# jmaronas/TGP.pytorch

Measured on AMD Instinct MI355X. Metric: ELBO-steps/sec (N x M kernel + chol + flow), Power M=100 S=32, higher is better.
Workload: dtype f64; 1 GPU; tgp_power_tanh3x2; rows_per_gpu=8611, D=4, M=100, S=32, flow=tanh3x2, parallelism=row-shard x1, launch=hipgraph, 40 / 10 steps per graph launch, replicas=1

## Files before the change

include/tgp_hip.h:

```cpp
#ifndef TGP_HIP_H
#define TGP_HIP_H

#include <stddef.h>
#include <stdint.h>

#ifdef __cplusplus
extern "C" {
#endif

#define TGP_VERSION 104
#define TGP_FUSED_MAX_M 128
#define TGP_BIG_MAX_M 4096

#define TGP_E_UNSUPPORTED (-100)
#define TGP_E_WORKSPACE (-101)
#define TGP_E_LDS (-102)
#define TGP_E_LAUNCH (-103)
#define TGP_E_COMM (-104)
#define TGP_STATUS_SYNC_TIMEOUT (-77)

#define TGP_FLOW_AFFINE 0
#define TGP_FLOW_SAL 1
#define TGP_FLOW_STEPTANH 2
#define TGP_FLOW_ARCSINH 3
#define TGP_FLOW_BOXCOX 4
#define TGP_FLOW_INV_BOXCOX 5
#define TGP_FLAG_RESTRICT 1
#define TGP_FLAG_ADD_F0 2
#define TGP_FLAG_PER_ROW 4

#define TGP_LIK_GAUSS 0
#define TGP_LIK_FLOW 1
#define TGP_LIK_ADJOINT 2
#define TGP_LIK_BERNOULLI 3
#define TGP_LIK_WARPED 4
#define TGP_LIK_SOFTMAX 5

#define TGP_KERNEL_SCALE_RBF 0
#define TGP_KERNEL_SCALE_MATERN32 1

#define TGP_PLAN_ROWS_AUTO 0
#define TGP_PLAN_ROWS_K16 1
#define TGP_PLAN_ROWS_K 2
#define TGP_PLAN_ROWS4_NW4 3
#define TGP_PLAN_ROWS4_NW8 4
#define TGP_PLAN_ROWS_MASK 15
#define TGP_PLAN_NO_CHUNK_OVERLAP 16
#define TGP_PLAN_CHUNK_ROWS(n) (((((n) + 127) / 128) & 0xffff) << 8)
#define TGP_PLAN_CHUNK_OF(plan) ((((plan) >> 8) & 0xffff) * 128)

typedef struct tgp_model {
  int32_t N;
  int32_t D;
  int32_t M;
  int32_t S;
  int32_t nblk;
  int32_t P;
  int32_t RP;
  int32_t lik;
  int32_t kernel;
  int32_t plan;
  double scale;
  double jitter;
  double kl_scale;
  double jitter_ladder;
  const double* Z;
  const double* raw_ls;
  const double* raw_os;
  const double* m;
  const double* Lam;
  const double* log_var_noise;
  const double* theta;
  const int32_t* program;
  const double* xs;
  const double* wn;
} tgp_model;

typedef struct tgp_grads {
  double* Z;
  double* raw_ls;
// ... 178 lines not shown
```

tgp/pytorch_amd/csrc/tgp_dev.hpp:

```cpp
#pragma once
#include <utility>
#include <hip/hip_runtime.h>
#include <stdint.h>
#include "../../../include/tgp_hip.h"

typedef double d4 __attribute__((ext_vector_type(4)));
#define TGP_MFMA(a, b, c) __builtin_amdgcn_mfma_f64_16x16x4f64((a), (b), (c), 0, 0, 0)

#define TGP_ROWS_PER_BLOCK 64
#define TGP_TILE_LD 66
#define TGP_MAX_MT 8
#ifndef TGP_RSPLIT
#define TGP_RSPLIT 4
#endif
#define TGP_LOG_2PI_REF 1.8378770942368803

#ifdef TGP_STAMPS
#define TGP_STAMP(wsp, plan, i)                                                                       \
  do {                                                                                                \
    if (blockIdx.x == 0 && threadIdx.x == 0)                                                          \
      (wsp)[(plan).hdr + tgp::H_STAMP + (i)] = (double)__builtin_amdgcn_s_memrealtime();              \
  } while (0)
#else
#define TGP_STAMP(wsp, plan, i) \
  do {                          \
  } while (0)
#endif

namespace tgp {

__device__ __forceinline__ void st_wt(double* p, double v) {
  __hip_atomic_store(p, v, __ATOMIC_RELAXED, __HIP_MEMORY_SCOPE_AGENT);
}

struct Plan {
  int N, D, M, S, nblk, P, RP, lik;
  int MT, MP, DP, CT, CT16, ntri, nblocks;
  int nw4;
  int rw;
  int rpb;
  int nslots;
  int zs_lds;
  size_t slab_G, slab_T, slab_S, slab_C, slab_len;
  size_t hdr, ils, ls, Zs, mpad, w, tp, tg;
  size_t Kmm, L, J, LT, Lq, LqT, S_, HpT, Q;
  size_t nD;
  size_t Gp;
  size_t redp;
  size_t PP;
  int PPW;
  size_t dbg;
  size_t slabs;
  size_t total;
};

enum { H_S2 = 0, H_KL = 1, H_ETA = 2, H_EINV = 3, H_SIG_OS = 4, H_STEP = 5, H_STAMP = 8, H_PSTAMP = 32, H_OUT = 60, H_N = 64 };
enum { C_ELL = 0, C_ETAB = 1, C_SVB = 2, C_PAD = 3, C_THETA = 4 };

inline size_t rup(size_t x, size_t a) { return (x + a - 1) / a * a; }

inline int rows4_waves(int N, int MT) {
  if ((N + 15) / 16 + MT <= 255) return 4;
  if ((N + 31) / 32 + MT <= 255) return 8;
  return 0;
}
inline int rows_rw(int N) { return (N > 4000 && (N + 39) / 40 <= 256) ? 10 : 16; }
inline int plan_alloc_blocks(int N) {
  int nb = (N + TGP_ROWS_PER_BLOCK - 1) / TGP_ROWS_PER_BLOCK;
  const int nw = rows4_waves(N, 1);
  if (nw > 0 && (N + 4 * nw - 1) / (4 * nw) > nb) nb = (N + 4 * nw - 1) / (4 * nw);
  const int rw = rows_rw(N);
  if ((N + 4 * rw - 1) / (4 * rw) > nb) nb = (N + 4 * rw - 1) / (4 * rw);
  return nb < 1 ? 1 : nb;
}

inline int make_plan(Plan& p, int N, int D, int M, int S, int nblk, int P, int RP, int lik, int nw4 = 0, int rw = 16) {
  if (D < 1 || D > 16) return -2;
  if (M < 1 || M > 16 * TGP_MAX_MT) return TGP_E_UNSUPPORTED;
  p.N = N; p.D = D; p.M = M; p.S = S; p.nblk = nblk; p.P = P; p.RP = RP; p.lik = lik; p.nslots = 0; p.zs_lds = 0;
  p.MT = (M + 15) / 16; p.MP = p.MT * 16;
  p.DP = D <= 4 ? 4 : (D <= 8 ? 8 : 16);
  p.CT = (2 * p.DP + 1 + 15) / 16; p.CT16 = p.CT * 16;
  p.ntri = p.MT * (p.MT + 1) / 2;
  p.nw4 = nw4;
  p.rw = rw;
  p.rpb = nw4 > 0 ? 4 * nw4 : 4 * rw;
  p.nblocks = (N + p.rpb - 1) / p.rpb;
  if (p.nblocks < 1) p.nblocks = 1;
  p.slab_G = 0;
  p.slab_T = p.slab_G + (size_t)p.ntri * 256;
  p.slab_S = p.slab_T + (size_t)p.MP * p.CT16;
  p.slab_C = p.slab_S + p.MP;
  p.slab_len = rup(p.slab_C + C_THETA + P, 16);
  size_t o = 0;
  const size_t mm = (size_t)p.MP * p.MP;
  p.hdr = o; o += H_N;
  p.ils = o; o += 16;
  p.ls = o; o += 16;
  p.Zs = o; o += (size_t)p.MP * p.DP;
  p.mpad = o; o += p.MP;
  p.w = o; o += p.MP;
  p.tp = o; o += rup(P + 1, 16);
  p.tg = o; o += rup(P + 1, 16);
  p.Kmm = o; o += mm; p.L = o; o += mm; p.J = o; o += mm; p.LT = o; o += mm;
  p.Lq = o; o += mm; p.LqT = o; o += mm; p.S_ = o; o += mm; p.HpT = o; o += mm; p.Q = o; o += mm;
  p.nD = o; o += (size_t)p.MT * 256;
  p.Gp = o; o += mm;
  p.redp = o; o += p.slab_len;
  p.PPW = p.DP + 2;
  p.PP = o; o += (size_t)2 * p.MT * p.MP * p.PPW;
  p.dbg = o; o += 256;
  p.slabs = o; o += (size_t)p.nblocks * p.slab_len;
  p.total = o;
  return 0;
}


__device__ __forceinline__ double exp_fast(double x) {
  x = fmin(fmax(x, -745.0), 709.0);
  const double k = rint(x * 1.4426950408889634074);
  double r = fma(-k, 6.93147180369123816490e-01, x);
  r = fma(-k, 1.90821492927058770002e-10, r);
  const double r2 = r * r, r4 = r2 * r2, r8 = r4 * r4;
  const double p01 = 1.0 + r;
  const double p23 = fma(r, 1.0 / 6.0, 0.5);
  const double p45 = fma(r, 1.0 / 120.0, 1.0 / 24.0);
  const double p67 = fma(r, 1.0 / 5040.0, 1.0 / 720.0);
  const double p89 = fma(r, 1.0 / 362880.0, 1.0 / 40320.0);
  const double pab = fma(r, 1.0 / 39916800.0, 1.0 / 3628800.0);
  const double pcd = fma(r, 1.0 / 6227020800.0, 1.0 / 479001600.0);
  const double q0 = fma(p23, r2, p01), q1 = fma(p67, r2, p45), q2 = fma(pab, r2, p89);
  const double s0 = fma(q1, r4, q0), s1 = fma(pcd, r4, q2);
  return ldexp(fma(s1, r8, s0), (int)k);
}

#define TGP_SQRT3 1.7320508075688772
__device__ __forceinline__ double cov_value(int kernel, double s2, double d2) {
  if (kernel == TGP_KERNEL_SCALE_MATERN32) {
    const double ar = TGP_SQRT3 * sqrt(fmax(d2, 1e-30));
    return s2 * (1.0 + ar) * exp_fast(-ar);
  }
  return s2 * exp_fast(-0.5 * d2);
}
__device__ __forceinline__ double cov_gweight(int kernel, double s2, double d2) {
// ... 1025 lines not shown
```

tgp/pytorch_amd/csrc/tgp_mm.hip:

```cpp
#include "tgp_dev.hpp"
#include "tgp_prep.hpp"
#include "tgp_launch.hpp"

namespace tgp {

#define PREP_THREADS 512
#ifndef TGP_W4_WINDOWS
#define TGP_W4_WINDOWS 2
#endif

__global__ __launch_bounds__(PREP_THREADS) void k_prep_a(Plan p, tgp_model md, FlowProg fp, double* __restrict__ ws,
                                                         int32_t* __restrict__ status) {
  extern __shared__ __attribute__((aligned(16))) unsigned char smem_raw[];
  double* sm = reinterpret_cast<double*>(smem_raw);
  const int tid = threadIdx.x, lane = tid & 63;
  const int wave = __builtin_amdgcn_readfirstlane(tid >> 6);
  const int r = lane & 15, q = lane >> 4;
  const int M = p.M, D = p.D, MP = p.MP, DP = p.DP, MT = p.MT;

  int32_t* sy = status + 4;
  const int nb_total = 3 + MT * MT;
  if ((int)blockIdx.x < MT * MT) {
    prep_tile_role<PREP_THREADS, true>(p, md, ws, (int)blockIdx.x, sy);
    sync_leave(sy, nb_total);
// ... 251 lines not shown
    __syncthreads();
    if (s_info == 0 || s_nan != 0 || !(md.jitter_ladder > 0.0) || attempt == 3) break;
    __syncthreads();
    if (tid == 0) s_info = 0;
    jit = md.jitter + md.jitter_ladder * (attempt == 0 ? 1.0 : (attempt == 1 ? 10.0 : 100.0));
    __syncthreads();
  }
  if (((MT - 1) & 1) == cb && wave == NW - 1) inv_diag(MT - 1);
  for (int t = wave; t < (MT + 1 - cb) / 2; t += NW) write_L(MT - 1, 2 * t + cb);
  PSTAMP(9);
#ifdef TGP_STAMPS
  if (lane == 0) {
    if (wave == 0)
      for (int i = 0; i < 10; ++i) ws[p.hdr + H_PSTAMP + i] = tph[i];
    if (wave == 3) for (int i = 1; i <= 5; ++i) { ws[p.hdr + H_PSTAMP + 26 + i] = tph[i]; ws[p.hdr + 20 + i] = tcnt[i]; }
    ws[p.hdr + H_PSTAMP + 10 + 2 * wave] = tph[7];
    ws[p.hdr + H_PSTAMP + 11 + 2 * wave] = tph[8];
  }
#endif
  if (tid == 0 && cb == 0) {
    status[0] = s_sync != 0 ? TGP_STATUS_SYNC_TIMEOUT : s_info;
    if (s_sync != 0) __hip_atomic_fetch_add(status + 3, 1, __ATOMIC_RELAXED, __HIP_MEMORY_SCOPE_AGENT);
    status[1] = s_nan;
    status[2] = s_info == 0 ? attempt : 0;
  }
  sync_leave(sy, nb_total);
#undef PREP_BARRIER
}

size_t prep_a_lds_bytes(const Plan& p) {
  return ((size_t)p.MP * (p.MP + 1) + (p.zs_lds ? (size_t)p.MP * p.DP : 0) + 16) * sizeof(double);
}

#define RED_ELEMS (256 / TGP_RSPLIT)
__global__ __launch_bounds__(256) void k_reduce(Plan p, double* __restrict__ ws) {
#ifdef TGP_STAMPS
  if (blockIdx.x == 0 && threadIdx.x == 0) ws[p.dbg + 200 + 16] = (double)__builtin_amdgcn_s_memrealtime();
#endif
  __shared__ double part_s[TGP_RSPLIT][RED_ELEMS];
  const int tid = threadIdx.x, sh = tid / RED_ELEMS, el = tid % RED_ELEMS;
  const size_t e = (size_t)blockIdx.x * RED_ELEMS + el;
  const bool in = e < p.slab_len;
  const int b0 = (int)((long long)p.nblocks * sh / TGP_RSPLIT), b1 = (int)((long long)p.nblocks * (sh + 1) / TGP_RSPLIT);
  const double* sl = ws + p.slabs + (in ? e : 0);
  constexpr int RB = 28;
  double s0 = 0.0, s1 = 0.0, s2 = 0.0, s3 = 0.0;
  for (int b = b0; b < b1; b += RB) {
    double t[RB];
#pragma unroll
    for (int u = 0; u < RB; ++u) {
      const int bu = b + u < b1 ? b + u : b1 - 1;
      t[u] = sl[(size_t)bu * p.slab_len];
    }
#pragma unroll
    for (int u = 0; u < RB; ++u) t[u] = b + u < b1 ? t[u] : 0.0;
#pragma unroll
    for (int u = 0; u < RB; u += 4) { s0 += t[u]; s1 += t[u + 1]; s2 += t[u + 2]; s3 += t[u + 3]; }
  }
  part_s[sh][el] = b1 > b0 ? (s0 + s1) + (s2 + s3) : 0.0;
  __syncthreads();
  if (sh != 0 || !in) return;
  double s = 0.0;
#pragma unroll
  for (int k = 0; k < TGP_RSPLIT; ++k) s += part_s[k][el];
  if (e < p.slab_T) {
    const int t = (int)(e >> 8), in_t = (int)(e & 255), row = in_t >> 4, col = in_t & 15;
    int ti = 0;
    while ((ti + 1) * (ti + 2) / 2 <= t) ++ti;
    const int tj = t - ti * (ti + 1) / 2;
    if (ti == tj && col > row) return;
    double* G = ws + p.Gp;
// ... 64 lines not shown
  }
  sv0 = tid < 16 ? red_tail(p, ws, p.slab_S + c0 + tid) : 0.0;
}
__device__ __forceinline__ void bwd_g_commit(const Plan& p, double* Gs, double* LbL, double* svL,
                                             const bwd_d2 (&gv)[BWD_G_NIT], double sv0) {
  const int MP = p.MP, tid = threadIdx.x;
#pragma unroll
  for (int u = 0; u < BWD_G_NIT; ++u) {
    const int i = tid + u * BWD_THREADS;
    if (i < MP * 8) {
      reinterpret_cast<bwd_d2*>(Gs)[i] = gv[u];
      reinterpret_cast<bwd_d2*>(LbL)[i] = bwd_d2{0.0, 0.0};
    }
  }
  if (tid < 16) svL[tid] = sv0;
}

template <int PF, bool SWAP = false, class FB>
__device__ __forceinline__ d4 tile_mm_regA(const double (&a)[PF], FB fb, int n, d4 acc) {
#pragma unroll
  for (int s0 = 0; s0 < PF; s0 += 8) {
    if (s0 < n) {
      double o[8];
#pragma unroll
      for (int u = 0; u < 8; ++u) o[u] = s0 + u < n ? fb(s0 + u) : 0.0;
#pragma unroll
      for (int u = 0; u < 8; ++u)
        if (s0 + u < n) acc = SWAP ? TGP_MFMA(o[u], a[s0 + u], acc) : TGP_MFMA(a[s0 + u], o[u], acc);
    }
  }
  return acc;
}

__device__ __forceinline__ void bwd_lam_role(const Plan& p, const tgp_model& md, const tgp_grads& g, double* __restrict__ ws,
                                             const AdamDev& ad, double* sm, int c, const int32_t* __restrict__ status) {
  static_assert(TGP_MAX_MT <= BWD_THREADS / 64, "one tile per wave");
  const int MP = p.MP, MT = p.MT, M = p.M;
  double* Gs = sm;
  double* LbL = Gs + (size_t)MP * 16;
  double* svL = LbL + (size_t)MP * 16;
  const int tid = threadIdx.x, lane = tid & 63, wave = __builtin_amdgcn_readfirstlane(tid >> 6), r = lane & 15, q = lane >> 4;
  const int c0 = 16 * c;
  BW_STAMP(c == 0, 4);
  bwd_d2 gv[BWD_G_NIT];
  double sv0;
  bwd_g_issue(p, ws, c0, gv, sv0);
  constexpr int PF = TGP_PF2;
  const double* __restrict__ Lq = ws + p.Lq;
  const int j = wave, j0 = 16 * j;
  const bool has = j < MT;
  const int n = has && j <= c ? (MP - j0) / 4 : 0;
  double lq[PF];
#pragma unroll
  for (int s_ = 0; s_ < PF; ++s_) lq[s_] = s_ < n ? Lq[(size_t)(j0 + 4 * s_ + q) * MP + j0 + r] : 0.0;
  const bool upd = ad.p != nullptr && !bwd_timed_out(status);
  const double step = upd ? (double)(ad.step_dev[0] + 1) : 1.0;
  double lamv[4], am[4], av[4];
  long ei[4];
#pragma unroll
  for (int rr = 0; rr < 4; ++rr) {
    const int row = c0 + r, col = j0 + q + 4 * rr;
    const bool in = has && row < M && col < M;
    const size_t e = in ? (size_t)row * M + col : 0;
    ei[rr] = in ? (long)e : -1;
    lamv[rr] = md.Lam[e];
    if (upd) { am[rr] = ad.m[ad.lam_off + e]; av[rr] = ad.v[ad.lam_off + e]; }
  }
  bwd_g_commit(p, Gs, LbL, svL, gv, sv0);
  __syncthreads();
  d4 acc = {0, 0, 0, 0};
  acc = tile_mm_regA<PF>(lq, [&](int s_) { return Gs[(j0 + 4 * s_ + q) * 16 + r]; }, n, acc);
  const double bc1 = 1.0 - exp_fast(step * ad.ln_b1), bc2s = sqrt(1.0 - exp_fast(step * ad.ln_b2));
#pragma unroll
  for (int rr = 0; rr < 4; ++rr) {
    if (ei[rr] < 0) continue;
    const int row = c0 + r, col = j0 + q + 4 * rr;
    double x = 0.0;
    if (col <= row) x = 2.0 * acc[rr] - md.kl_scale * (col == row ? lamv[rr] - 1.0 / lamv[rr] : lamv[rr]);
    g.Lam[ei[rr]] = x;
    if (upd) adam_elem(ad, ad.lam_off + ei[rr], x, ad.p[ad.lam_off + ei[rr]], am[rr], av[rr], bc1, bc2s);
  }
  BW_STAMP(c == 0, 5);
}

__device__ __forceinline__ void bwd_q_role(const Plan& p, double* __restrict__ ws, double* sm, int c, int32_t* sb) {
  static_assert(TGP_MAX_MT <= BWD_THREADS / 64, "one tile per wave");
  const int MP = p.MP, MT = p.MT;
  double* Gs = sm;
  double* LbL = Gs + (size_t)MP * 16;
  double* svL = LbL + (size_t)MP * 16;
  const int tid = threadIdx.x, lane = tid & 63, wave = __builtin_amdgcn_readfirstlane(tid >> 6), r = lane & 15, q = lane >> 4;
  const int c0 = 16 * c;
  BW_STAMP(c == 0, 0);
  bwd_d2 gv[BWD_G_NIT];
  double sv0;
  bwd_g_issue(p, ws, c0, gv, sv0);
  constexpr int PF = TGP_PF2;
  const double* __restrict__ HpT = ws + p.HpT;
  const double* __restrict__ Lm = ws + p.L;
  const double* __restrict__ w = ws + p.w;
  const bool has = wave < MT - c;
  const bool spare = MT - c < BWD_THREADS / 64, tw = spare && wave == MT - c;
  const int i0 = tw ? c0 : 16 * (c + wave);
  const int n1 = has ? MP / 4 : 0, n2 = has || tw ? (MP - i0) / 4 : 0;
  double hp[PF], pq[PF], wv[4];
#pragma unroll
  for (int s_ = 0; s_ < PF; ++s_) hp[s_] = s_ < n1 ? HpT[(size_t)(4 * s_ + q) * MP + i0 + r] : 0.0;
#pragma unroll
  for (int s_ = 0; s_ < PF; ++s_) pq[s_] = s_ < n2 ? Lm[(size_t)(i0 + 4 * s_ + q) * MP + i0 + r] : 0.0;
#pragma unroll
  for (int rr = 0; rr < 4; ++rr) wv[rr] = has ? w[i0 + q + 4 * rr] : 0.0;
  bwd_g_commit(p, Gs, LbL, svL, gv, sv0);
  __syncthreads();
  BW_STAMP(c == 0, 1);
  if (has) {
    d4 acc = {0, 0, 0, 0};
    acc = tile_mm_regA<PF>(hp, [&](int s_) { return Gs[(4 * s_ + q) * 16 + r]; }, n1, acc);
#pragma unroll
    for (int rr = 0; rr < 4; ++rr) {
      const int row = i0 + q + 4 * rr, col = c0 + r;
      LbL[row * 16 + r] = (col <= row) ? -(wv[rr] * svL[r] + 2.0 * acc[rr]) : 0.0;
    }
  }
  __syncthreads();
  BW_STAMP(c == 0, 2);
  double* Q = ws + p.Q;
  if (has) {
    d4 acc = {0, 0, 0, 0};
    acc = tile_mm_regA<PF>(pq, [&](int s_) { return LbL[(i0 + 4 * s_ + q) * 16 + r]; }, n2, acc);
    if (wave != 0) {
#pragma unroll
      for (int rr = 0; rr < 4; ++rr) {
        const int row = i0 + q + 4 * rr, col = c0 + r;
        st_agent(Q + (size_t)row * MP + col, acc[rr]);
        st_agent(Q + (size_t)col * MP + row, acc[rr]);
      }
    } else {
      d4 tr = {0, 0, 0, 0};
      if (!spare) tr = tile_mm_regA<PF, true>(pq, [&](int s_) { return LbL[(c0 + 4 * s_ + q) * 16 + r]; }, n2, tr);
#pragma unroll
      for (int rr = 0; rr < 4; ++rr) {
        const int rl = q + 4 * rr;
        if (r <= rl) st_agent(Q + (size_t)(c0 + rl) * MP + c0 + r, acc[rr]);
        else if (!spare) st_agent(Q + (size_t)(c0 + rl) * MP + c0 + r, tr[rr]);
      }
    }
  } else if (tw) {
    d4 tr = {0, 0, 0, 0};
    tr = tile_mm_regA<PF, true>(pq, [&](int s_) { return LbL[(c0 + 4 * s_ + q) * 16 + r]; }, n2, tr);
#pragma unroll
    for (int rr = 0; rr < 4; ++rr) {
      const int rl = q + 4 * rr;
      if (r > rl) st_agent(Q + (size_t)(c0 + rl) * MP + c0 + r, tr[rr]);
    }
  }
  handoff_barrier();
  if (tid == 0) sync_add(sb + SB_PROG, 1 << 16);
  BW_STAMP(c == 0, 3);
}

__device__ __forceinline__ void bwd_row_role(const Plan& p, double* __restrict__ ws, double* sm, int i, int h, int32_t* sb,
                                             int32_t* __restrict__ status) {
  static_assert(TGP_MAX_MT <= BWD_THREADS / 64, "one Y tile and one Ks tile per wave");
  const int MP = p.MP, MT = p.MT, DP = p.DP, PPW = p.PPW;
  const int tid = threadIdx.x, lane = tid & 63, wave = __builtin_amdgcn_readfirstlane(tid >> 6), r = lane & 15, q = lane >> 4;
  const int KH = (MT + 1) / 2, kb0 = h ? KH : 0, kb1 = h ? MT : KH, nk = kb1 - kb0;
  double* Yl = sm;
  double* zsL = Yl + (size_t)MT * 256;
  double* Ja = zsL + 16 * DP;
  const int i0 = 16 * i;
  const double* __restrict__ J = ws + p.J;
  const double* __restrict__ Q = ws + p.Q;
  BW_STAMP(i == 0 && h == 0, 6);
  double kmv[4];
  const int jbw = wave < MT ? wave : 0, j0w = 16 * jbw;
#pragma unroll
  for (int rr = 0; rr < 4; ++rr) kmv[rr] = (ws + p.Kmm)[(size_t)(i0 + q + 4 * rr) * MP + j0w + r];
  if (tid < 16 * DP) zsL[tid] = (ws + p.Zs)[(size_t)i0 * DP + tid];
  for (int e = tid; e < (MP - i0) * 16; e += BWD_THREADS) Ja[e] = J[(size_t)(i0 + (e >> 4)) * MP + i0 + (e & 15)];
  const int ks0 = 16 * (jbw > kb0 ? jbw : kb0), ks1 = 16 * kb1;
  const int n1 = wave < nk ? (MP - i0) / 4 : 0, n2 = wave < MT && ks1 > ks0 ? (ks1 - ks0) / 4 : 0;
  constexpr int PF = TGP_PF2, PFH = 2 * TGP_MAX_MT;
  double jb2[PFH];
#pragma unroll
  for (int s_ = 0; s_ < PFH; ++s_) jb2[s_] = s_ < n2 ? J[(size_t)(ks0 + 4 * s_ + q) * MP + j0w + r] : 0.0;
  __syncthreads();
  BW_STAMP(i == 0 && h == 0, 7);
  bwd_wait(sb + SB_PROG, [&](int x) { return ((x >> 16) & 0xff) >= MT; }, status);
  BW_STAMP(i == 0 && h == 0, 8);
  if (wave < nk) {
    d4 acc = {0, 0, 0, 0};
    double qv[PF];
#pragma unroll
    for (int s_ = 0; s_ < PF; ++s_) qv[s_] = s_ < n1 ? ld_agent(Q + (size_t)(i0 + 4 * s_ + q) * MP + 16 * (kb0 + wave) + r) : 0.0;
    acc = tile_mm_regA<PF, true>(qv, [&](int s_) { return Ja[(4 * s_ + q) * 16 + r]; }, n1, acc);
#pragma unroll
    for (int rr = 0; rr < 4; ++rr) Yl[wave * 256 + (q + 4 * rr) * 16 + r] = acc[rr];
  }
  __syncthreads();
  BW_STAMP(i == 0 && h == 0, 9);
  if (wave < MT) {
    d4 acc = {0, 0, 0, 0};
    acc = tile_mm_regA<PFH, true>(jb2, [&](int s_) { const int k = ks0 + 4 * s_; return Yl[((k >> 4) - kb0) * 256 + r * 16 + (k & 15) + q]; }, n2, acc);
    double ep[4];
#pragma unroll
    for (int rr = 0; rr < 4; ++rr) ep[rr] = 0.5 * acc[rr] * kmv[rr];
    double cs = quad_sum((ep[0] + ep[1]) + (ep[2] + ep[3]));
    double* out = ws + p.PP + (size_t)(2 * i + h) * PPW * MP + j0w + r;
    if (q == 0) st_agent(out + (size_t)DP * MP, cs);
    for (int d = 0; d < DP; ++d) {
      double s = 0.0;
#pragma unroll
      for (int rr = 0; rr < 4; ++rr) s += ep[rr] * zsL[(q + 4 * rr) * DP + d];
      s = quad_sum(s);
      if (q == 0) st_agent(out + (size_t)d * MP, s);
    }
  }
  handoff_barrier();
  if (tid == 0) sync_add(sb + SB_PROG, 1 << 24);
  BW_STAMP(i == 0 && h == 0, 10);
}

#define BWD_MIRROR_MAX 4096
#define BWDF_ADAM_PER_THREAD 2
__device__ __forceinline__ void bwd_final_role(const Plan& p, const tgp_model& md, const tgp_grads& g, double* __restrict__ out,
                                               double* __restrict__ ws, const AdamDev& ad, double* term, int32_t* sb,
                                               int32_t* __restrict__ status, int nb_total) {
// ... 92 lines not shown
      out[1] = timed_out ? nan_ : ell;
      out[2] = timed_out ? nan_ : kl;
      out[3] = 0.0;
    }
  }
  if (ad.p != nullptr && !timed_out) {
    if (mirror) __syncthreads();
    else handoff_barrier();
    const double bc1 = 1.0 - exp_fast(a_step * ad.ln_b1), bc2s = sqrt(1.0 - exp_fast(a_step * ad.ln_b2));
    auto grad = [&](long k, long i) { return mirror ? gl[k] : __hip_atomic_load(ad.g + i, __ATOMIC_RELAXED, __HIP_MEMORY_SCOPE_AGENT); };
#pragma unroll
    for (int u = 0; u < BWDF_ADAM_PER_THREAD; ++u) {
      const long k = tid + (long)NT * u;
      if (k < n_rest) {
        const long i = k < ad.lam_off ? k : k + ad.lam_n;
        adam_elem(ad, i, grad(k, i), ap[u], am[u], av[u], bc1, bc2s);
      }
    }
    for (long k = tid + (long)NT * BWDF_ADAM_PER_THREAD; k < n_rest; k += NT) {
      const long i = k < ad.lam_off ? k : k + ad.lam_n;
      adam_elem(ad, i, grad(k, i), ad.p[i], ad.m[i], ad.v[i], bc1, bc2s);
    }
  }
  BW_STAMP(true, 14);
  bwd_wait(sb + SB_LEFT, [&](int x) { return x >= nb_total - 1; }, status);
  __syncthreads();
  if (tid == 0) {
    sync_st(sb + SB_PROG, 0); sync_st(sb + SB_LEFT, 0);
    if (ad.p != nullptr && !timed_out) atomicAdd(&ad.step_dev[0], 1);
  }
  BW_STAMP(true, 15);
}

__global__ __launch_bounds__(BWD_THREADS) void k_bwd(Plan p, tgp_model md, tgp_grads g, double* __restrict__ out,
                                                     double* __restrict__ ws, AdamDev ad, int32_t* __restrict__ status) {
  extern __shared__ __attribute__((aligned(16))) unsigned char smem_raw[];
  double* sm = reinterpret_cast<double*>(smem_raw);
  const int MT = p.MT, b = (int)blockIdx.x;
  int32_t* sb = status + 6;
  if (b < MT) {
    bwd_q_role(p, ws, sm, b, sb);
    bwd_leave(sb);
  } else if (b < 2 * MT) {
    bwd_lam_role(p, md, g, ws, ad, sm, b - MT, status);
    bwd_leave(sb);
  } else if (b < 4 * MT) {
    bwd_row_role(p, ws, sm, (b - 2 * MT) >> 1, (b - 2 * MT) & 1, sb, status);
    bwd_leave(sb);
  } else {
    bwd_final_role(p, md, g, out, ws, ad, sm, sb, status, 4 * MT + 1);
  }
}

#define COV_ROWS 64
#define COV_COLS 128
__global__ __launch_bounds__(256) void k_cov_tile(int kernel, const double* __restrict__ X1, int N1,
                                                   const double* __restrict__ X2, int N2, int D,
                                                   const double* __restrict__ raw_ls, const double* __restrict__ raw_os,
                                                   double jitter, int self, double* __restrict__ K) {
  __shared__ double xl[COV_ROWS * 16];
  __shared__ double ils[17];
  const int tid = threadIdx.x, cp = tid & 63, rg = tid >> 6;
  const long n0 = (long)blockIdx.x * COV_ROWS;
  const int m0 = blockIdx.y * COV_COLS + 2 * cp;
  if (tid < 16) ils[tid] = tid < D ? 1.0 / softplus_d(raw_ls[tid]) : 0.0;
  if (tid == 64) ils[16] = softplus_d(raw_os[0]);
  double z0[16], z1[16];
  {
    const long ma = m0 < N2 ? m0 : N2 - 1, mb = m0 + 1 < N2 ? m0 + 1 : N2 - 1;
#pragma unroll
    for (int d = 0; d < 16; ++d) {
      z0[d] = d < D ? X2[ma * D + d] : 0.0;
      z1[d] = d < D ? X2[mb * D + d] : 0.0;
    }
  }
  const long nrem = (long)N1 - n0, nr = nrem < COV_ROWS ? nrem : COV_ROWS;
  double xv[4];
#pragma unroll
  for (int u = 0; u < 4; ++u) {
    const int i = tid + 256 * u;
    xv[u] = i < nr * D ? X1[n0 * D + i] : 0.0;
  }
  __syncthreads();
  const double s2 = ils[16];
// ... 196 lines not shown
  for (int i = tid; i < M * M; i += PREP_THREADS) {
    const int r = i / M, c = i % M;
    double l = 0.0, jv = 0.0;
    if (c < r) { l = A[r * LD + c]; jv = A[c * LD + r]; }
    else if (c == r) { l = A[r * LD + r]; jv = dinv[r]; }
    Lout[i] = l;
    if (Jout != nullptr) Jout[i] = jv;
  }
  if (tid == 0) { status[0] = s_info; status[1] = s_nan; }
}

#define LAUNCH_CHECK()                                   \
  do {                                                   \
    hipError_t e_ = hipGetLastError();                   \
    if (e_ != hipSuccess) return set_error(e_, __FILE__, __LINE__); \
  } while (0)

int launch_prepare(const Plan& p_in, const tgp_model& md, const FlowProg& fp, double* ws, int32_t* status,
                   hipStream_t st) {
  Plan p = p_in;
  p.zs_lds = 1;
  if (prep_a_lds_bytes(p) > 160 * 1024 - 1024) p.zs_lds = 0;
  const size_t lds = prep_a_lds_bytes(p);
  static size_t lds_cur = 48 * 1024;
  if (int rc = ensure_lds(reinterpret_cast<const void*>(k_prep_a), lds, &lds_cur)) return rc;
  hipLaunchKernelGGL(k_prep_a, dim3(3 + p.MT * p.MT), dim3(PREP_THREADS), lds, st, p, md, fp, ws, status);
  LAUNCH_CHECK();
  return 0;
}

int launch_backward_mm(const Plan& p, const tgp_model& md, const tgp_grads& g, double* out, double* ws, int32_t* status,
                       hipStream_t st, const AdamDev* adam) {
  const AdamDev ad = adam != nullptr ? *adam : AdamDev();
  hipLaunchKernelGGL(k_reduce, dim3((unsigned)((p.slab_len + RED_ELEMS - 1) / RED_ELEMS)), dim3(256), 0, st, p, ws);
  LAUNCH_CHECK();
  const size_t lds_col = (size_t)(2 * p.MP * 16 + 16), lds_row = (size_t)p.MT * 256 + 16 * p.DP + (size_t)p.MP * 16,
               lds_fin = (size_t)p.M * (p.D + 1) + (adam != nullptr && ad.n - ad.lam_n <= BWD_MIRROR_MAX ? (size_t)(ad.n - ad.lam_n) : 0) + p.M;
  const size_t lds = sizeof(double) * (lds_col > lds_row ? (lds_col > lds_fin ? lds_col : lds_fin) : (lds_row > lds_fin ? lds_row : lds_fin));
  hipLaunchKernelGGL(k_bwd, dim3(4 * p.MT + 1), dim3(BWD_THREADS), lds, st, p, md, g, out, ws, ad, status);
  LAUNCH_CHECK();
  return 0;
}

static int launch_cov_tile(int kernel, const double* X1, int N1, const double* X2, int N2, int D, const double* raw_ls,
                           const double* raw_os, double jitter, int self, double* K, hipStream_t st) {
  if (D < 1 || D > 16) return TGP_E_UNSUPPORTED;
  if (N1 < 1 || N2 < 1) return 0;
  if ((N2 & 1) == 0 && N2 >= 2 && (long)N2 * D <= 4096 && N2 <= 512 && (reinterpret_cast<uintptr_t>(K) & 15) == 0) {
    const unsigned gx = (unsigned)((N1 + COVF_ROWS - 1) / COVF_ROWS);
    const size_t lds = ((size_t)D * N2 + (size_t)D * COVF_ROWS) * sizeof(double);
    static size_t lds_cur = 48 * 1024;
    if (int rc = ensure_lds(reinterpret_cast<const void*>(k_cov_flat), lds, &lds_cur)) return rc;
    hipLaunchKernelGGL(k_cov_flat, dim3(gx), dim3(256), lds, st, kernel, X1, N1, X2, N2, D, raw_ls, raw_os, jitter, self, K);
    LAUNCH_CHECK();
    return 0;
  }
  const unsigned gx = (unsigned)((N1 + COV_ROWS - 1) / COV_ROWS), gy = (unsigned)((N2 + COV_COLS - 1) / COV_COLS);
  if (gy > 65535u) return TGP_E_UNSUPPORTED;
  hipLaunchKernelGGL(k_cov_tile, dim3(gx, gy), dim3(256), 0, st, kernel, X1, N1, X2, N2, D, raw_ls, raw_os, jitter, self, K);
  LAUNCH_CHECK();
  return 0;
}

int launch_kmm(const double* Z, const double* raw_ls, const double* raw_os, int M, int D, double jitter, double* K,
               hipStream_t st) {
  return launch_cov_tile(TGP_KERNEL_SCALE_RBF, Z, M, Z, M, D, raw_ls, raw_os, jitter, 1, K, st);
}

int launch_knm(const double* X, const double* Z, const double* raw_ls, const double* raw_os, int N, int M, int D,
               double* K, hipStream_t st) {
  return launch_cov_tile(TGP_KERNEL_SCALE_RBF, X, N, Z, M, D, raw_ls, raw_os, 0.0, 0, K, st);
}
// ... 25 lines not shown
```

tgp/pytorch_amd/lib.py:

```python
import ctypes as C
import os

import torch

_HERE = os.path.dirname(os.path.abspath(__file__))
LIB_PATH = os.path.join(_HERE, "libtgp_hip.so")

FLOW_AFFINE, FLOW_SAL, FLOW_STEPTANH = 0, 1, 2
FLOW_ARCSINH, FLOW_BOXCOX, FLOW_INV_BOXCOX = 3, 4, 5
FLAG_RESTRICT, FLAG_ADD_F0, FLAG_PER_ROW = 1, 2, 4
LIK_GAUSS, LIK_FLOW = 0, 1
LIK_BERNOULLI = 3
LIK_WARPED = 4
LIK_SOFTMAX = 5
SOFTMAX_MAX_C, SOFTMAX_MAX_S = 32, 256
E_UNSUPPORTED = -100

_dp = C.c_void_p


KERNEL_SCALE_RBF, KERNEL_SCALE_MATERN32 = 0, 1
KERNELS = {"scale_rbf": KERNEL_SCALE_RBF, "scale_matern32": KERNEL_SCALE_MATERN32}
PLAN_ROWS_AUTO, PLAN_ROWS_K16, PLAN_ROWS_K, PLAN_ROWS4_NW4, PLAN_ROWS4_NW8 = 0, 1, 2, 3, 4
PLAN_NO_CHUNK_OVERLAP = 16


def plan_chunk_rows(n):
    return (((int(n) + 127) // 128) & 0xffff) << 8


class TgpModel(C.Structure):
    _fields_ = [("N", C.c_int32), ("D", C.c_int32), ("M", C.c_int32), ("S", C.c_int32), ("nblk", C.c_int32),
                ("P", C.c_int32), ("RP", C.c_int32), ("lik", C.c_int32), ("kernel", C.c_int32), ("plan", C.c_int32),
                ("scale", C.c_double),
                ("jitter", C.c_double), ("kl_scale", C.c_double), ("jitter_ladder", C.c_double), ("Z", _dp), ("raw_ls", _dp), ("raw_os", _dp),
                ("m", _dp), ("Lam", _dp), ("log_var_noise", _dp), ("theta", _dp), ("program", _dp), ("xs", _dp),
                ("wn", _dp)]


class TgpGrads(C.Structure):
    _fields_ = [("Z", _dp), ("raw_ls", _dp), ("raw_os", _dp), ("m", _dp), ("Lam", _dp), ("log_var_noise", _dp),
                ("theta", _dp), ("rowp", _dp)]


class TgpAdamArgs(C.Structure):
    _fields_ = [("params", _dp), ("grads", _dp), ("exp_avg", _dp), ("exp_avg_sq", _dp), ("n", C.c_int64), ("lr", C.c_double),
                ("beta1", C.c_double), ("beta2", C.c_double), ("eps", C.c_double), ("step_dev", _dp), ("maximize", C.c_int32),
                ("phases", C.c_uint32)]


class TgpMlp(C.Structure):
    _fields_ = [("N", C.c_int32), ("D", C.c_int32), ("H", C.c_int32), ("L", C.c_int32), ("nnets", C.c_int32),
                ("act", C.c_int32), ("training", C.c_int32), ("reserved0", C.c_int32), ("drop_p", C.c_double),
                ("seed", C.c_uint64)]


class TgpSoftmax(C.Structure):
# ... 132 lines not shown
```

Baseline: 10660 ELBO-steps/s.

## Pre-pack backward matrices into MFMA fragment image layout during reduce

After: 10690 ELBO-steps/s, median of 6. Within noise of the previous version (+0.3%).

```diff
diff --git a/include/tgp_hip.h b/include/tgp_hip.h
--- a/include/tgp_hip.h
+++ b/include/tgp_hip.h
@@ -46,6 +46,7 @@
 #define TGP_PLAN_ROWS4_NW8 4
 #define TGP_PLAN_ROWS_MASK 15
 #define TGP_PLAN_NO_CHUNK_OVERLAP 16
+#define TGP_PLAN_BWD_ROWMAJOR 32
 #define TGP_PLAN_CHUNK_ROWS(n) (((((n) + 127) / 128) & 0xffff) << 8)
 #define TGP_PLAN_CHUNK_OF(plan) ((((plan) >> 8) & 0xffff) * 128)
 
diff --git a/tgp/pytorch_amd/csrc/tgp_dev.hpp b/tgp/pytorch_amd/csrc/tgp_dev.hpp
--- a/tgp/pytorch_amd/csrc/tgp_dev.hpp
+++ b/tgp/pytorch_amd/csrc/tgp_dev.hpp
@@ -52,12 +52,18 @@
   size_t dbg;
   size_t slabs;
   size_t total;
+  size_t Li, Lqi, Ji, HpTi;
 };
 
 enum { H_S2 = 0, H_KL = 1, H_ETA = 2, H_EINV = 3, H_SIG_OS = 4, H_STEP = 5, H_STAMP = 8, H_PSTAMP = 32, H_OUT = 60, H_N = 64 };
 enum { C_ELL = 0, C_ETAB = 1, C_SVB = 2, C_PAD = 3, C_THETA = 4 };
 
 inline size_t rup(size_t x, size_t a) { return (x + a - 1) / a * a; }
+
+__host__ __device__ inline size_t bwd_img_pair(int MP, int b, int u, int l) { return (((size_t)b * (MP / 8) + u) * 64 + l) * 2; }
+__host__ __device__ inline size_t bwd_img_elem(int MP, int k, int col) {
+  return bwd_img_pair(MP, col >> 4, k >> 3, 16 * (k & 3) + (col & 15)) + ((k >> 2) & 1);
+}
 
 inline int rows4_waves(int N, int MT) {
   if ((N + 15) / 16 + MT <= 255) return 4;
@@ -110,6 +116,7 @@
   p.PPW = p.DP + 2;
   p.PP = o; o += (size_t)2 * p.MT * p.MP * p.PPW;
   p.dbg = o; o += 256;
+  p.Li = o; o += mm; p.Lqi = o; o += mm; p.Ji = o; o += mm; p.HpTi = o; o += mm;
   p.slabs = o; o += (size_t)p.nblocks * p.slab_len;
   p.total = o;
   return 0;
diff --git a/tgp/pytorch_amd/csrc/tgp_mm.hip b/tgp/pytorch_amd/csrc/tgp_mm.hip
--- a/tgp/pytorch_amd/csrc/tgp_mm.hip
+++ b/tgp/pytorch_amd/csrc/tgp_mm.hip
@@ -307,11 +307,37 @@
   return ((size_t)p.MP * (p.MP + 1) + (p.zs_lds ? (size_t)p.MP * p.DP : 0) + 16) * sizeof(double);
 }
 
+typedef double red_d2 __attribute__((ext_vector_type(2)));
+#define RED_IMG_PAIRS ((2 * TGP_MAX_MT + 3) / 4)
+__device__ __forceinline__ void reduce_image_role(const Plan& p, double* __restrict__ ws, int x) {
+  const int MP = p.MP, MT = p.MT, m = x / MT, b = x - m * MT;
+  const size_t src = m == 0 ? p.L : m == 1 ? p.Lq : m == 2 ? p.J : p.HpT;
+  const size_t dst = m == 0 ? p.Li : m == 1 ? p.Lqi : m == 2 ? p.Ji : p.HpTi;
+  const int lane = threadIdx.x & 63, wave = threadIdx.x >> 6, r = lane & 15, q = lane >> 4;
+  const int u0 = (m == 3 ? 0 : 2 * b) + wave, nu = MP / 8;
+  red_d2 v[RED_IMG_PAIRS];
+#pragma unroll
+  for (int k = 0; k < RED_IMG_PAIRS; ++k) {
+    const int u = u0 + 4 * k < nu ? u0 + 4 * k : nu - 1;
+    const double* xp = ws + src + (size_t)(8 * u + q) * MP + 16 * b + r;
+    v[k] = red_d2{xp[0], xp[(size_t)4 * MP]};
+  }
+#pragma unroll
+  for (int k = 0; k < RED_IMG_PAIRS; ++k) {
+    const int u = u0 + 4 * k;
+    if (u < nu) *reinterpret_cast<red_d2*>(ws + dst + bwd_img_pair(MP, b, u, lane)) = v[k];
+  }
+}
+
 #define RED_ELEMS (256 / TGP_RSPLIT)
-__global__ __launch_bounds__(256) void k_reduce(Plan p, double* __restrict__ ws) {
+__global__ __launch_bounds__(256) void k_reduce(Plan p, double* __restrict__ ws, int nred, int images) {
 #ifdef TGP_STAMPS
   if (blockIdx.x == 0 && threadIdx.x == 0) ws[p.dbg + 200 + 16] = (double)__builtin_amdgcn_s_memrealtime();
 #endif
+  if ((int)blockIdx.x >= nred) {
+    if (images) reduce_image_role(p, ws, (int)blockIdx.x - nred);
+    return;
+  }
   __shared__ double part_s[TGP_RSPLIT][RED_ELEMS];
   const int tid = threadIdx.x, sh = tid / RED_ELEMS, el = tid % RED_ELEMS;
   const size_t e = (size_t)blockIdx.x * RED_ELEMS + el;
@@ -442,6 +468,25 @@
   return acc;
 }
 
+template <int PF>
+__device__ __forceinline__ void bwd_img_frags(const double* __restrict__ img, int MP, int b, int u0, int lane, int n, double (&a)[PF]) {
+  static_assert(PF % 2 == 0, "pairs of k-steps");
+  const bwd_d2* __restrict__ ip = reinterpret_cast<const bwd_d2*>(img + bwd_img_pair(MP, b, u0, lane));
+#pragma unroll
+  for (int u = 0; u < PF / 2; ++u) {
+    bwd_d2 v = {0.0, 0.0};
+    if (2 * u < n) v = ip[(size_t)u * 64];
+    a[2 * u] = v[0];
+    a[2 * u + 1] = v[1];
+  }
+}
+__device__ __forceinline__ bwd_d2 ld_agent2(ws_rsrc_t rs, size_t off) {
+  typedef unsigned u4v __attribute__((ext_vector_type(4)));
+  const u4v v = __builtin_amdgcn_raw_buffer_load_b128(rs, (int)(off * 8), 0, 16);
+  return bwd_d2{__hiloint2double((int)v[1], (int)v[0]), __hiloint2double((int)v[3], (int)v[2])};
+}
+
+template <bool IMG>
 __device__ __forceinline__ void bwd_lam_role(const Plan& p, const tgp_model& md, const tgp_grads& g, double* __restrict__ ws,
                                              const AdamDev& ad, double* sm, int c, const int32_t* __restrict__ status) {
   static_assert(TGP_MAX_MT <= BWD_THREADS / 64, "one tile per wave");
@@ -461,8 +506,12 @@
   const bool has = j < MT;
   const int n = has && j <= c ? (MP - j0) / 4 : 0;
   double lq[PF];
-#pragma unroll
-  for (int s_ = 0; s_ < PF; ++s_) lq[s_] = s_ < n ? Lq[(size_t)(j0 + 4 * s_ + q) * MP + j0 + r] : 0.0;
+  if constexpr (IMG) {
+    bwd_img_frags<PF>(ws + p.Lqi, MP, j, j0 / 8, lane, n, lq);
+  } else {
+#pragma unroll
+    for (int s_ = 0; s_ < PF; ++s_) lq[s_] = s_ < n ? Lq[(size_t)(j0 + 4 * s_ + q) * MP + j0 + r] : 0.0;
+  }
   const bool upd = ad.p != nullptr && !bwd_timed_out(status);
   const double step = upd ? (double)(ad.step_dev[0] + 1) : 1.0;
   double lamv[4], am[4], av[4];
@@ -493,6 +542,7 @@
   BW_STAMP(c == 0, 5);
 }
 
+template <bool IMG>
 __device__ __forceinline__ void bwd_q_role(const Plan& p, double* __restrict__ ws, double* sm, int c, int32_t* sb) {
   static_assert(TGP_MAX_MT <= BWD_THREADS / 64, "one tile per wave");
   const int MP = p.MP, MT = p.MT;
@@ -514,10 +564,15 @@
   const int i0 = tw ? c0 : 16 * (c + wave);
   const int n1 = has ? MP / 4 : 0, n2 = has || tw ? (MP - i0) / 4 : 0;
   double hp[PF], pq[PF], wv[4];
-#pragma unroll
-  for (int s_ = 0; s_ < PF; ++s_) hp[s_] = s_ < n1 ? HpT[(size_t)(4 * s_ + q) * MP + i0 + r] : 0.0;
-#pragma unroll
-  for (int s_ = 0; s_ < PF; ++s_) pq[s_] = s_ < n2 ? Lm[(size_t)(i0 + 4 * s_ + q) * MP + i0 + r] : 0.0;
+  if constexpr (IMG) {
+    bwd_img_frags<PF>(ws + p.HpTi, MP, i0 >> 4, 0, lane, n1, hp);
+    bwd_img_frags<PF>(ws + p.Li, MP, i0 >> 4, i0 / 8, lane, n2, pq);
+  } else {
+#pragma unroll
+    for (int s_ = 0; s_ < PF; ++s_) hp[s_] = s_ < n1 ? HpT[(size_t)(4 * s_ + q) * MP + i0 + r] : 0.0;
+#pragma unroll
+    for (int s_ = 0; s_ < PF; ++s_) pq[s_] = s_ < n2 ? Lm[(size_t)(i0 + 4 * s_ + q) * MP + i0 + r] : 0.0;
+  }
 #pragma unroll
   for (int rr = 0; rr < 4; ++rr) wv[rr] = has ? w[i0 + q + 4 * rr] : 0.0;
   bwd_g_commit(p, Gs, LbL, svL, gv, sv0);
@@ -535,15 +590,25 @@
   __syncthreads();
   BW_STAMP(c == 0, 2);
   double* Q = ws + p.Q;
+  auto q_at = [&](int row, int col) { return IMG ? bwd_img_elem(MP, row, col) : (size_t)row * MP + col; };
   if (has) {
     d4 acc = {0, 0, 0, 0};
     acc = tile_mm_regA<PF>(pq, [&](int s_) { return LbL[(i0 + 4 * s_ + q) * 16 + r]; }, n2, acc);
     if (wave != 0) {
-#pragma unroll
-      for (int rr = 0; rr < 4; ++rr) {
-        const int row = i0 + q + 4 * rr, col = c0 + r;
-        st_agent(Q + (size_t)row * MP + col, acc[rr]);
-        st_agent(Q + (size_t)col * MP + row, acc[rr]);
+      if constexpr (IMG) {
+        const ws_rsrc_t rs = ws_rsrc(ws);
+        const size_t o = p.Q + bwd_img_pair(MP, c, i0 / 8, lane);
+        st_agent2(rs, o, acc[0], acc[1]);
+        st_agent2(rs, o + 128, acc[2], acc[3]);
+#pragma unroll
+        for (int rr = 0; rr < 4; ++rr) st_agent(Q + bwd_img_elem(MP, c0 + r, i0 + q + 4 * rr), acc[rr]);
+      } else {
+#pragma unroll
+        for (int rr = 0; rr < 4; ++rr) {
+          const int row = i0 + q + 4 * rr, col = c0 + r;
+          st_agent(Q + (size_t)row * MP + col, acc[rr]);
+          st_agent(Q + (size_t)col * MP + row, acc[rr]);
+        }
       }
     } else {
       d4 tr = {0, 0, 0, 0};
@@ -551,8 +616,8 @@
 #pragma unroll
       for (int rr = 0; rr < 4; ++rr) {
         const int rl = q + 4 * rr;
-        if (r <= rl) st_agent(Q + (size_t)(c0 + rl) * MP + c0 + r, acc[rr]);
-        else if (!spare) st_agent(Q + (size_t)(c0 + rl) * MP + c0 + r, tr[rr]);
+        if (r <= rl) st_agent(Q + q_at(c0 + rl, c0 + r), acc[rr]);
+        else if (!spare) st_agent(Q + q_at(c0 + rl, c0 + r), tr[rr]);
       }
     }
   } else if (tw) {
@@ -561,7 +626,7 @@
 #pragma unroll
     for (int rr = 0; rr < 4; ++rr) {
       const int rl = q + 4 * rr;
-      if (r > rl) st_agent(Q + (size_t)(c0 + rl) * MP + c0 + r, tr[rr]);
+      if (r > rl) st_agent(Q + q_at(c0 + rl, c0 + r), tr[rr]);
     }
   }
   handoff_barrier();
@@ -569,6 +634,7 @@
   BW_STAMP(c == 0, 3);
 }
 
+template <bool IMG>
 __device__ __forceinline__ void bwd_row_role(const Plan& p, double* __restrict__ ws, double* sm, int i, int h, int32_t* sb,
                                              int32_t* __restrict__ status) {
   static_assert(TGP_MAX_MT <= BWD_THREADS / 64, "one Y tile and one Ks tile per wave");
@@ -587,13 +653,34 @@
 #pragma unroll
   for (int rr = 0; rr < 4; ++rr) kmv[rr] = (ws + p.Kmm)[(size_t)(i0 + q + 4 * rr) * MP + j0w + r];
   if (tid < 16 * DP) zsL[tid] = (ws + p.Zs)[(size_t)i0 * DP + tid];
-  for (int e = tid; e < (MP - i0) * 16; e += BWD_THREADS) Ja[e] = J[(size_t)(i0 + (e >> 4)) * MP + i0 + (e & 15)];
+  static_assert(2 * (BWD_THREADS / 64) * 8 >= 16 * TGP_MAX_MT, "two pairs per thread cover the MP / 8 pairs of a block column");
+  bwd_d2 jv[2];
+  if constexpr (IMG) {
+    const bwd_d2* __restrict__ ip = reinterpret_cast<const bwd_d2*>(ws + p.Ji + bwd_img_pair(MP, i, i0 / 8, lane));
+#pragma unroll
+    for (int u = 0; u < 2; ++u) {
+      const int up = (tid >> 6) + 8 * u;
+      jv[u] = bwd_d2{0.0, 0.0};
+      if (8 * up < MP - i0) jv[u] = ip[(size_t)up * 64];
+    }
+  } else {
+    for (int e = tid; e < (MP - i0) * 16; e += BWD_THREADS) Ja[e] = J[(size_t)(i0 + (e >> 4)) * MP + i0 + (e & 15)];
+  }
   const int ks0 = 16 * (jbw > kb0 ? jbw : kb0), ks1 = 16 * kb1;
   const int n1 = wave < nk ? (MP - i0) / 4 : 0, n2 = wave < MT && ks1 > ks0 ? (ks1 - ks0) / 4 : 0;
   constexpr int PF = TGP_PF2, PFH = 2 * TGP_MAX_MT;
   double jb2[PFH];
-#pragma unroll
-  for (int s_ = 0; s_ < PFH; ++s_) jb2[s_] = s_ < n2 ? J[(size_t)(ks0 + 4 * s_ + q) * MP + j0w + r] : 0.0;
+  if constexpr (IMG) {
+    bwd_img_frags<PFH>(ws + p.Ji, MP, jbw, ks0 / 8, lane, n2, jb2);
+#pragma unroll
+    for (int u = 0; u < 2; ++u) {
+      const int up = (tid >> 6) + 8 * u;
+      if (8 * up < MP - i0) { Ja[(8 * up + q) * 16 + r] = jv[u][0]; Ja[(8 * up + 4 + q) * 16 + r] = jv[u][1]; }
+    }
+  } else {
+#pragma unroll
+    for (int s_ = 0; s_ < PFH; ++s_) jb2[s_] = s_ < n2 ? J[(size_t)(ks0 + 4 * s_ + q) * MP + j0w + r] : 0.0;
+  }
   __syncthreads();
   BW_STAMP(i == 0 && h == 0, 7);
   bwd_wait(sb + SB_PROG, [&](int x) { return ((x >> 16) & 0xff) >= MT; }, status);
@@ -601,8 +688,20 @@
   if (wave < nk) {
     d4 acc = {0, 0, 0, 0};
     double qv[PF];
-#pragma unroll
-    for (int s_ = 0; s_ < PF; ++s_) qv[s_] = s_ < n1 ? ld_agent(Q + (size_t)(i0 + 4 * s_ + q) * MP + 16 * (kb0 + wave) + r) : 0.0;
+    if constexpr (IMG) {
+      const ws_rsrc_t rs = ws_rsrc(ws);
+      const size_t o = p.Q + bwd_img_pair(MP, kb0 + wave, i0 / 8, lane);
+#pragma unroll
+      for (int u = 0; u < PF / 2; ++u) {
+        bwd_d2 v = {0.0, 0.0};
+        if (2 * u < n1) v = ld_agent2(rs, o + (size_t)u * 128);
+        qv[2 * u] = v[0];
+        qv[2 * u + 1] = v[1];
+      }
+    } else {
+#pragma unroll
+      for (int s_ = 0; s_ < PF; ++s_) qv[s_] = s_ < n1 ? ld_agent(Q + (size_t)(i0 + 4 * s_ + q) * MP + 16 * (kb0 + wave) + r) : 0.0;
+    }
     acc = tile_mm_regA<PF, true>(qv, [&](int s_) { return Ja[(4 * s_ + q) * 16 + r]; }, n1, acc);
 #pragma unroll
     for (int rr = 0; rr < 4; ++rr) Yl[wave * 256 + (q + 4 * rr) * 16 + r] = acc[rr];
@@ -761,24 +860,33 @@
   BW_STAMP(true, 15);
 }
 
-__global__ __launch_bounds__(BWD_THREADS) void k_bwd(Plan p, tgp_model md, tgp_grads g, double* __restrict__ out,
-                                                     double* __restrict__ ws, AdamDev ad, int32_t* __restrict__ status) {
+template <bool IMG>
+__device__ __forceinline__ void bwd_body(const Plan& p, const tgp_model& md, const tgp_grads& g, double* __restrict__ out,
+                                         double* __restrict__ ws, const AdamDev& ad, int32_t* __restrict__ status) {
   extern __shared__ __attribute__((aligned(16))) unsigned char smem_raw[];
   double* sm = reinterpret_cast<double*>(smem_raw);
   const int MT = p.MT, b = (int)blockIdx.x;
   int32_t* sb = status + 6;
   if (b < MT) {
-    bwd_q_role(p, ws, sm, b, sb);
+    bwd_q_role<IMG>(p, ws, sm, b, sb);
     bwd_leave(sb);
   } else if (b < 2 * MT) {
-    bwd_lam_role(p, md, g, ws, ad, sm, b - MT, status);
+    bwd_lam_role<IMG>(p, md, g, ws, ad, sm, b - MT, status);
     bwd_leave(sb);
   } else if (b < 4 * MT) {
-    bwd_row_role(p, ws, sm, (b - 2 * MT) >> 1, (b - 2 * MT) & 1, sb, status);
+    bwd_row_role<IMG>(p, ws, sm, (b - 2 * MT) >> 1, (b - 2 * MT) & 1, sb, status);
     bwd_leave(sb);
   } else {
     bwd_final_role(p, md, g, out, ws, ad, sm, sb, status, 4 * MT + 1);
   }
+}
+__global__ __launch_bounds__(BWD_THREADS) void k_bwd(Plan p, tgp_model md, tgp_grads g, double* __restrict__ out,
+                                                     double* __restrict__ ws, AdamDev ad, int32_t* __restrict__ status) {
+  bwd_body<true>(p, md, g, out, ws, ad, status);
+}
+__global__ __launch_bounds__(BWD_THREADS) void k_bwd_rm(Plan p, tgp_model md, tgp_grads g, double* __restrict__ out,
+                                                        double* __restrict__ ws, AdamDev ad, int32_t* __restrict__ status) {
+  bwd_body<false>(p, md, g, out, ws, ad, status);
 }
 
 #define COV_ROWS 64
@@ -1041,12 +1149,16 @@
 int launch_backward_mm(const Plan& p, const tgp_model& md, const tgp_grads& g, double* out, double* ws, int32_t* status,
                        hipStream_t st, const AdamDev* adam) {
   const AdamDev ad = adam != nullptr ? *adam : AdamDev();
-  hipLaunchKernelGGL(k_reduce, dim3((unsigned)((p.slab_len + RED_ELEMS - 1) / RED_ELEMS)), dim3(256), 0, st, p, ws);
+  const int nred = (int)((p.slab_len + RED_ELEMS - 1) / RED_ELEMS), images = (md.plan & TGP_PLAN_BWD_ROWMAJOR) ? 0 : 1;
+  hipLaunchKernelGGL(k_reduce, dim3((unsigned)(nred + (images ? 4 * p.MT : 0))), dim3(256), 0, st, p, ws, nred, images);
   LAUNCH_CHECK();
   const size_t lds_col = (size_t)(2 * p.MP * 16 + 16), lds_row = (size_t)p.MT * 256 + 16 * p.DP + (size_t)p.MP * 16,
                lds_fin = (size_t)p.M * (p.D + 1) + (adam != nullptr && ad.n - ad.lam_n <= BWD_MIRROR_MAX ? (size_t)(ad.n - ad.lam_n) : 0) + p.M;
   const size_t lds = sizeof(double) * (lds_col > lds_row ? (lds_col > lds_fin ? lds_col : lds_fin) : (lds_row > lds_fin ? lds_row : lds_fin));
-  hipLaunchKernelGGL(k_bwd, dim3(4 * p.MT + 1), dim3(BWD_THREADS), lds, st, p, md, g, out, ws, ad, status);
+  if (md.plan & TGP_PLAN_BWD_ROWMAJOR)
+    hipLaunchKernelGGL(k_bwd_rm, dim3(4 * p.MT + 1), dim3(BWD_THREADS), lds, st, p, md, g, out, ws, ad, status);
+  else
+    hipLaunchKernelGGL(k_bwd, dim3(4 * p.MT + 1), dim3(BWD_THREADS), lds, st, p, md, g, out, ws, ad, status);
   LAUNCH_CHECK();
   return 0;
 }
diff --git a/tgp/pytorch_amd/lib.py b/tgp/pytorch_amd/lib.py
--- a/tgp/pytorch_amd/lib.py
+++ b/tgp/pytorch_amd/lib.py
@@ -23,6 +23,7 @@
 KERNELS = {"scale_rbf": KERNEL_SCALE_RBF, "scale_matern32": KERNEL_SCALE_MATERN32}
 PLAN_ROWS_AUTO, PLAN_ROWS_K16, PLAN_ROWS_K, PLAN_ROWS4_NW4, PLAN_ROWS4_NW8 = 0, 1, 2, 3, 4
 PLAN_NO_CHUNK_OVERLAP = 16
+PLAN_BWD_ROWMAJOR = 32
 
 
 def plan_chunk_rows(n):
```
